# wenet-e2e/wenet

Measured on AMD Instinct MI355X. Metric: audio-seconds/sec (RTF^-1), 12L Conformer fbank80, ctc_prefix_beam_search, higher is better.
Workload: dtype f32 (feed-forward and subsampling-conv2 GEMMs: fp32 operands as three exact bf16 planes, six plane products on the bf16 matrix cores, f32 accumulate -- error <= the v_mfma_f32 kernel's, tests/test_gpu_x6.py; everything else v_mfma_f32)

## Files before the change

### wenet_amd/csrc/ffn_x6f.hip

```cpp
#include <type_traits>

#include "common.h"
#include "gemm_epilogue.h"
#include "kernels.h"
#include "x6.h"

namespace wn {

namespace {

__device__ unsigned long long g_x6f_clk[4][24];

constexpr int REC = X3_REC;
constexpr int XSTAGE = 24 * REC;
constexpr int XD = 256;
constexpr int XKB = XD / 16;

typedef unsigned u32x4 __attribute__((ext_vector_type(4)));
struct Frag6 { bf16x8 p[2][3]; };

__global__ __launch_bounds__(256) void x6_split_perm_kernel(const float* __restrict__ src, int R,
                                                            int K, int ld,
                                                            char* __restrict__ dst) {
  const int tiles = (R + 31) >> 5, nkb = K >> 4;
  const int64_t idx = (int64_t)blockIdx.x * 256 + threadIdx.x;
  const int row_l = (int)(idx & 31), h = (int)((idx >> 5) & 1);
  const int64_t rest = idx >> 6;
  const int kb = (int)(rest % nkb), tile = (int)(rest / nkb);
  if (tile >= tiles) return;
  const int row = tile * 32 + row_l;
  f32x4 a = {0.f, 0.f, 0.f, 0.f}, b = a;
  if (row < R) {
    const float* s = src + (int64_t)row * ld + kb * 16 + h * 4;
    a = *reinterpret_cast<const f32x4*>(s);
    b = *reinterpret_cast<const f32x4*>(s + 8);
  }
  bf16x8 p0, p1, p2;
#pragma unroll
  for (int e = 0; e < 4; ++e) {
    const Split3 sa = split3(a[e]), sb = split3(b[e]);
    p0[e] = sa.h0; p1[e] = sa.h1; p2[e] = sa.h2;
    p0[4 + e] = sb.h0; p1[4 + e] = sb.h1; p2[4 + e] = sb.h2;
  }
  char* o = dst + ((int64_t)kb * tiles + tile) * X3_TILE + h * 512 + row_l * 16;
  *reinterpret_cast<bf16x8*>(o) = p0;
  *reinterpret_cast<bf16x8*>(o + REC) = p1;
  *reinterpret_cast<bf16x8*>(o + 2 * REC) = p2;
}

__device__ __forceinline__ void wait_vm_stages(int stages) {
  switch (stages) {
    case 0: asm volatile("s_waitcnt vmcnt(0)" ::: "memory"); break;
    case 1: asm volatile("s_waitcnt vmcnt(6)" ::: "memory"); break;
    case 2: asm volatile("s_waitcnt vmcnt(12)" ::: "memory"); break;
    case 3: asm volatile("s_waitcnt vmcnt(18)" ::: "memory"); break;
    default: asm volatile("s_waitcnt vmcnt(24)" ::: "memory"); break;
  }
}

template <int ACT, int RING, int VAR>
__global__ __launch_bounds__(256, 1) void ffn_x6f_kernel(FfnX6Args p, int tiles_m, int pairmap) {
  extern __shared__ __attribute__((aligned(16))) char smem_g[];
  typedef __attribute__((address_space(3))) void* lds_ptr;
  constexpr int HALF = (VAR & 512) ? 2 : 1;
  constexpr int STG = XSTAGE * HALF;
  constexpr int SPC = 8 / HALF;
  static_assert(RING >= 3 && RING * STG <= 6 * XSTAGE, "ring of at most 144 KB");
  float* b1s = reinterpret_cast<float*>(smem_g + RING * STG);

  const int bid = blockIdx.x, xcd = bid & 7, rr = bid >> 3;
  int slice, tm;
  if (pairmap && p.S >= 2 && p.S <= 8) {
    const int nsp = p.S >> 1, pair = xcd % nsp, tg = xcd / nsp;
    slice = 2 * pair + (rr & 1);
    tm = (rr >> 1) * (8 / nsp) + tg;
  } else if (p.S <= 8) {
    slice = xcd & (p.S - 1);
    tm = rr * (8 / p.S) + xcd / p.S;
  } else {
    const int sub = p.S >> 3;
    slice = xcd + 8 * (rr % sub);
    tm = rr / sub;
  }
  if (tm >= tiles_m) return;

  unsigned long long clk[20] = {0, 0, 0, 0, 0, 0, 0, 0, 0, 0, 0, 0, 0, 0, 0, 0, 0, 0, 0, 0};
  if constexpr ((VAR & 8192) != 0) {
    clk[9] = __builtin_readcyclecounter();
    clk[12] = __builtin_amdgcn_s_memrealtime();
  }
  const int tid = threadIdx.x, lane = tid & 63;
  const int wave = __builtin_amdgcn_readfirstlane(tid >> 6);
  __builtin_assume(wave >= 0 && wave < 4);
  const int hi = lane >> 5, li = lane & 31;
  const int NC = p.F / p.S / 64;
  const int cg0 = slice * NC;
  const int FT = p.F >> 5;
  const unsigned vlane = (unsigned)lane * 16u;

  const __amdgpu_buffer_rsrc_t r1 = __builtin_amdgcn_make_buffer_rsrc(
      const_cast<char*>(reinterpret_cast<const char*>(p.W13)), 0,
      (int)((int64_t)p.F * XD * 6), 0x00020000);
  const __amdgpu_buffer_rsrc_t r2 = __builtin_amdgcn_make_buffer_rsrc(
      const_cast<char*>(reinterpret_cast<const char*>(p.W2p)), 0,
      (int)((int64_t)p.F * XD * 6), 0x00020000);

  auto issue_sub = [&](int c, int sub, int buf) {
    char* dst = smem_g + buf * STG + (sub % HALF) * XSTAGE + wave * 6 * REC;
    const int cg = cg0 + c;
    if (sub < 4) {
      const int nt = sub >> 1;
#pragma unroll
      for (int j2 = 0; j2 < 2; ++j2) {
        const int ks = (sub & 1) * 8 + wave * 2 + j2;
        const int so = ((ks * FT + 2 * cg + nt) * 3) * REC;
#pragma unroll
        for (int pl = 0; pl < 3; ++pl)
          __builtin_amdgcn_raw_ptr_buffer_load_lds(r1, (lds_ptr)(dst + (j2 * 3 + pl) * REC), 16,
                                                   vlane, so + pl * REC, 0, 0);
      }
    } else {
      const int so = ((cg * 4 + sub - 4) * 24 + wave * 6) * REC;
#pragma unroll
      for (int j = 0; j < 6; ++j)
        __builtin_amdgcn_raw_ptr_buffer_load_lds(r2, (lds_ptr)(dst + j * REC), 16, vlane,
                                                 so + j * REC, 0, 0);
    }
  };
  auto issue = [&](int c, int st, int buf) {
#pragma unroll
    for (int h = 0; h < HALF; ++h) issue_sub(c, st * HALF + h, buf);
  };
  auto issue_one = [&](int c, int sub, int buf, int j) {
    char* dst = smem_g + buf * STG + (sub % HALF) * XSTAGE + wave * 6 * REC + j * REC;
    const int cg = cg0 + c;
    if (sub < 4) {
      const int nt = sub >> 1, j2 = j / 3, pl = j - j2 * 3;
      const int ks = (sub & 1) * 8 + wave * 2 + j2;
      const int so = ((ks * FT + 2 * cg + nt) * 3) * REC;
      __builtin_amdgcn_raw_ptr_buffer_load_lds(r1, (lds_ptr)dst, 16, vlane, so + pl * REC, 0, 0);
    } else {
      const int so = ((cg * 4 + sub - 4) * 24 + wave * 6) * REC;
      __builtin_amdgcn_raw_ptr_buffer_load_lds(r2, (lds_ptr)dst, 16, vlane, so + j * REC, 0, 0);
    }
  };
  auto read_group = [&](int buf, int g) {
    const char* st = smem_g + buf * STG + g * 6 * REC + lane * 16;
    Frag6 f;
#pragma unroll
    for (int t = 0; t < 2; ++t)
#pragma unroll
      for (int pl = 0; pl < 3; ++pl)
        f.p[t][pl] = *reinterpret_cast<const bf16x8*>(st + (t * 3 + pl) * REC);
    return f;
  };

  constexpr bool XT = (VAR & 16384) != 0;
  constexpr bool XI = (VAR & 32768) != 0;
  bf16x8 X[XKB][3];
  const int xrow = min(tm * 128 + wave * 32 + li, p.M - 1);
  f32x4 xa[XKB], xb[XKB];
  f32x4 xr[4][8];
  if constexpr (XI) {
    const int tiles = (p.M + 31) >> 5;
    const int tile = min(tm * 4 + wave, tiles - 1);
    const char* xi = reinterpret_cast<const char*>(p.X3) + (int64_t)tile * X3_TILE + lane * 16;
    const int64_t kstr = (int64_t)tiles * X3_TILE;
#pragma unroll
    for (int ks = 0; ks < XKB; ++ks)
#pragma unroll
      for (int pl = 0; pl < 3; ++pl)
        X[ks][pl] = *reinterpret_cast<const bf16x8*>(xi + ks * kstr + pl * REC);
  } else if constexpr (XT) {
    const int r4 = lane >> 4, c16 = lane & 15;
#pragma unroll
    for (int q = 0; q < 4; ++q)
#pragma unroll
      for (int j = 0; j < 8; ++j) {
        const int row = min(tm * 128 + wave * 32 + 4 * j + r4, p.M - 1);
        xr[q][j] = *reinterpret_cast<const f32x4*>(p.X + (int64_t)row * p.ldx + q * 64 + c16 * 4);
      }
  } else {
    const float* xr0 = p.X + (int64_t)xrow * p.ldx + hi * 8;
#pragma unroll
    for (int ks = 0; ks < XKB; ++ks) {
      xa[ks] = *reinterpret_cast<const f32x4*>(xr0 + ks * 16);
      xb[ks] = *reinterpret_cast<const f32x4*>(xr0 + ks * 16 + 4);
    }
  }
#pragma unroll
  for (int t = 0; t < ((VAR & 16384) ? RING - 1 : RING); ++t) issue(0, t, t);
  float b1v[8];
#pragma unroll
  for (int i = 0; i < 8; ++i) b1v[i] = p.b1[cg0 * 64 + min(tid + 256 * i, NC * 64 - 1)];
  if constexpr ((VAR & 8192) != 0) { __builtin_amdgcn_sched_barrier(0); clk[15] = __builtin_readcyclecounter(); __builtin_amdgcn_sched_barrier(0); }
  if constexpr (XT && !XI) {
    char* patch = smem_g + (RING - 1) * STG + wave * (32 * 272);
    const int r4 = lane >> 4, c16 = lane & 15;
#pragma unroll
    for (int q = 0; q < 4; ++q) {
#pragma unroll
      for (int j = 0; j < 8; ++j)
        *reinterpret_cast<f32x4*>(patch + (4 * j + r4) * 272 + c16 * 16) = xr[q][j];
#pragma unroll
      for (int k4 = 0; k4 < 4; ++k4) {
        xa[4 * q + k4] = *reinterpret_cast<const f32x4*>(patch + li * 272 + k4 * 64 + hi * 32);
        xb[4 * q + k4] = *reinterpret_cast<const f32x4*>(patch + li * 272 + k4 * 64 + hi * 32 + 16);
      }
      asm volatile("s_waitcnt lgkmcnt(0)" ::: "memory");
    }
  }
  if constexpr (!XI) {
#pragma unroll
    for (int ks = 0; ks < XKB; ++ks) {
#pragma unroll
      for (int e = 0; e < 4; ++e) {
        const Split3 sa = split3(xa[ks][e]), sb = split3(xb[ks][e]);
        X[ks][0][e] = sa.h0; X[ks][1][e] = sa.h1; X[ks][2][e] = sa.h2;
        X[ks][0][4 + e] = sb.h0; X[ks][1][4 + e] = sb.h1; X[ks][2][4 + e] = sb.h2;
      }
    }
  }
  if constexpr ((VAR & 8192) != 0) { __builtin_amdgcn_sched_barrier(0); clk[16] = __builtin_readcyclecounter(); __builtin_amdgcn_sched_barrier(0); }
  asm volatile("s_waitcnt vmcnt(0)" ::: "memory");
  if constexpr ((VAR & 8192) != 0) { __builtin_amdgcn_sched_barrier(0); clk[17] = __builtin_readcyclecounter(); __builtin_amdgcn_sched_barrier(0); }
#pragma unroll
  for (int ks = 0; ks < XKB; ++ks)
#pragma unroll
    for (int pl = 0; pl < 3; ++pl) asm volatile("" : "+v"(X[ks][pl]));
#pragma unroll
  for (int i = 0; i < 8; ++i)
    if (tid + 256 * i < NC * 64) b1s[tid + 256 * i] = b1v[i];
  __syncthreads();
  if constexpr ((VAR & 8192) != 0) { __builtin_amdgcn_sched_barrier(0); clk[18] = __builtin_readcyclecounter(); __builtin_amdgcn_sched_barrier(0); }

  f32x16 Y[8];
#pragma unroll
  for (int i = 0; i < 8; ++i)
#pragma unroll
    for (int r = 0; r < 16; ++r) Y[i][r] = 0.f;
  f32x16 HE[2], HO[2];
  u32x4 Hp[4][3];
  if (VAR & 4)
#pragma unroll
    for (int i = 0; i < 12; ++i) {
      Hp[i / 3][i % 3] = u32x4{0x3f803f80u, 0x3f803f80u, 0x3f803f80u, 0x3f803f80u};
      asm volatile("" : "+v"(Hp[i / 3][i % 3]));
    }

  constexpr int PW[6] = {2, 0, 1, 1, 0, 0}, PX[6] = {0, 2, 1, 0, 1, 0};
  constexpr int RT[6] = {0, 1, 0, 1, 0, 1}, RP[6] = {2, 2, 0, 0, 1, 1};

  float pv0 = 0.f, pv1 = 0.f, pt0 = 0.f, pt1 = 0.f;
  unsigned ph0 = 0, ph1 = 0;
  auto pk = [](float a, float b) {
    typedef __bf16 bf16x2 __attribute__((ext_vector_type(2)));
    const bf16x2 h = {(__bf16)a, (__bf16)b};
    return __builtin_bit_cast(unsigned, h);
  };
  auto lo = [](unsigned u) { return __builtin_bit_cast(float, u << 16); };
  auto hi16 = [](unsigned u) { return __builtin_bit_cast(float, u & 0xffff0000u); };
  auto piece_slice = [&](int nt, int i, int k, const f32x4& bq) {
    const int r = 2 * i;
    switch (k) {
      case 0: {
        float b0 = bq[r & 3];
        asm volatile("" : "+v"(b0));
        pv0 = HE[nt][r] + b0;
        break;
      }
      case 1: {
        float b1 = bq[(r + 1) & 3];
        asm volatile("" : "+v"(b1), "+v"(pv0));
        pv0 += HO[nt][r];
        pv1 = HE[nt][r + 1] + b1;
        break;
      }
      case 2:
        asm volatile("" : "+v"(pv0), "+v"(pv1));
        pv1 += HO[nt][r + 1];
        if (ACT == ACT_SILU) pt0 = pv0 * -1.4426950408889634f;
        break;
      case 3:
        if (ACT == ACT_SILU) {
          asm volatile("" : "+v"(pt0), "+v"(pv1));
          pt1 = pv1 * -1.4426950408889634f;
          pt0 = wn_exp2(pt0);
        }
        break;
      case 4:
        if (ACT == ACT_SILU) {
          asm volatile("" : "+v"(pt0), "+v"(pt1));
          pt1 = wn_exp2(pt1);
          pt0 = 1.0f + pt0;
        }
        break;
      case 5:
        if (ACT == ACT_SILU) {
          asm volatile("" : "+v"(pt0), "+v"(pt1));
          pt1 = 1.0f + pt1;
          pt0 = wn_rcp(pt0);
        }
        break;
      case 6:
        asm volatile("" : "+v"(pv0));
        if (ACT == ACT_SILU) {
          asm volatile("" : "+v"(pt0), "+v"(pt1));
          pt1 = wn_rcp(pt1);
          pv0 *= pt0;
        }
        if (ACT == ACT_RELU) pv0 = fmaxf(pv0, 0.0f);
        break;
      case 7:
        asm volatile("" : "+v"(pv0), "+v"(pv1));
        if (ACT == ACT_SILU) {
          asm volatile("" : "+v"(pt1));
          pv1 *= pt1;
        }
        if (ACT == ACT_RELU) pv1 = fmaxf(pv1, 0.0f);
        ph0 = pk(pv0, pv1);
        break;
      case 8:
        asm volatile("" : "+v"(pv0), "+v"(pv1), "+v"(ph0));
        pv0 -= lo(ph0); pv1 -= hi16(ph0);
        break;
      case 9:
        asm volatile("" : "+v"(pv0), "+v"(pv1));
        ph1 = pk(pv0, pv1);
        break;
      case 10:
        asm volatile("" : "+v"(pv0), "+v"(pv1), "+v"(ph1));
        pv0 -= lo(ph1); pv1 -= hi16(ph1);
        break;
      default: {
        asm volatile("" : "+v"(pv0), "+v"(pv1));
        const int kb = 2 * nt + (r >> 3), d = (r & 7) >> 1;
        Hp[kb][0][d] = ph0;
        Hp[kb][1][d] = ph1;
        Hp[kb][2][d] = pk(pv0, pv1);
        break;
      }
    }
  };
  auto read_frag = [&](int b, int g, int t, int pl) {
    return *reinterpret_cast<const bf16x8*>(smem_g + b * STG + (g * 6 + t * 3 + pl) * REC +
                                            lane * 16);
  };
  const f32x16 zero16 = {0.f, 0.f, 0.f, 0.f, 0.f, 0.f, 0.f, 0.f, 0.f, 0.f, 0.f, 0.f, 0.f, 0.f, 0.f,
                         0.f};

  int buf = 0;
  Frag6 fc;
#pragma unroll
  for (int q = 0; q < 6; ++q) fc.p[RT[q]][RP[q]] = read_frag(0, 0, RT[q], RP[q]);
  if constexpr ((VAR & 8192) != 0) clk[10] = __builtin_readcyclecounter();
  auto chunk = [&](auto last_tag, int c) {
    constexpr bool last = decltype(last_tag)::value;
    f32x4 bq = {0.f, 0.f, 0.f, 0.f};
#pragma unroll
    for (int sub = 0; sub < 8; ++sub) {
      if constexpr ((VAR & 8192) != 0 && !last) {
        __builtin_amdgcn_sched_barrier(0);
        clk[sub] = __builtin_readcyclecounter();
        __builtin_amdgcn_sched_barrier(0);
      }
#pragma unroll
      for (int g = 0; g < 4; ++g) {
        Frag6 fn;
        const bool do_piece = sub >= 2 && sub < 6;
        const int pnt = sub >= 4 ? 1 : 0;
        const int pi = ((sub & 1) << 2) + g;
        if (do_piece && (pi & 1) == 0)
          bq = *reinterpret_cast<const f32x4*>(b1s + c * 64 + pnt * 32 + 8 * (pi >> 1) + 4 * hi);
#pragma unroll
        for (int k = 0; k < 12; ++k) {
          const int q = k >> 1, tl = k & 1;
          if ((VAR & 1) || ((VAR & 65536) && q >= 3)) {
            asm volatile("" ::"v"(fc.p[tl][PW[q]]));
          } else if (sub < 4) {
            const int nt = sub >> 1, ks = (sub & 1) * 8 + 2 * g + tl;
            const bool first = (sub & 1) == 0 && g == 0 && q == 0;
            f32x16& H = tl == 0 ? HE[nt] : HO[nt];
            H = __builtin_amdgcn_mfma_f32_32x32x16_bf16(fc.p[tl][PW[q]], X[ks][PX[q]],
                                                       first ? zero16 : H, 0, 0, 0);
          } else {
            const bf16x8 hb = __builtin_bit_cast(bf16x8, Hp[sub - 4][PX[q]]);
            Y[2 * g + tl] = __builtin_amdgcn_mfma_f32_32x32x16_bf16(fc.p[tl][PW[q]], hb,
                                                                    Y[2 * g + tl], 0, 0, 0);
          }
          const int st = sub / HALF;
          const bool sync_sub = sub % HALF == HALF - 1;
          const int gs = (sub % HALF) * 4 + g;
          if (g == 3 && k == 5 && sync_sub) {
            __builtin_amdgcn_sched_barrier(0);
            if (!(VAR & 8)) {
              if (!(VAR & 1024)) {
                asm volatile("s_waitcnt lgkmcnt(0)" ::: "memory");
                const int tail = SPC - 2 - st < 0 ? 0 : (SPC - 2 - st > RING - 2 ? RING - 2 : SPC - 2 - st);
                if (last) wait_vm_stages(tail * HALF); else wait_vm_stages((RING - 2) * HALF);
              }
              if (!(VAR & 2048)) __builtin_amdgcn_s_barrier();
            }
            if (!(VAR & 2) && !(VAR & 16384)) {
              if (st + RING < SPC) issue(c, st + RING, buf);
              else if (!last) issue(c + 1, st + RING - SPC, buf);
            }
            buf = buf + 1 == RING ? 0 : buf + 1;
            __builtin_amdgcn_sched_barrier(0);
          }
          if constexpr ((VAR & 16384) != 0 && !(VAR & 2)) {
            static_assert(!(VAR & 16384) || HALF == 2, "spread DMA: 48-record stages");
            const int ka = do_piece ? 9 : 2, kb = do_piece ? 11 : 8;
            if ((k == ka || k == kb) && gs < 6) {
              const int j12 = gs * 2 + (k == kb ? 1 : 0);
              const int tst = st + RING - 1;
              const int bufp = buf == 0 ? RING - 1 : buf - 1;
              if (tst < SPC) issue_one(c, tst * HALF + j12 / 6, bufp, j12 % 6);
              else if (!last) issue_one(c + 1, (tst - SPC) * HALF + j12 / 6, bufp, j12 % 6);
            }
          }
          if (VAR & 64) {
            fn = fc;
          } else if (g < 3 || !sync_sub) {
            if (VAR & 4096) {
              if (k == 0)
#pragma unroll
                for (int i = 0; i < 6; ++i) fn.p[RT[i]][RP[i]] = read_frag(buf, gs + 1, RT[i], RP[i]);
            } else if (tl == 1) {
              fn.p[RT[q]][RP[q]] = read_frag(buf, gs + 1, RT[q], RP[q]);
            }
          } else if (k >= 6 && (sub < 7 || !last)) {
            fn.p[RT[k - 6]][RP[k - 6]] = read_frag(buf, 0, RT[k - 6], RP[k - 6]);
          }
          if (do_piece) {
            if (VAR & 4) {
              if (k == 11) {
                const int r = 2 * pi, kb = 2 * pnt + (r >> 3), d = (r & 7) >> 1;
                Hp[kb][0][d] = __builtin_bit_cast(unsigned, HE[pnt][r]) & 0x3f803f80u;
                Hp[kb][1][d] = __builtin_bit_cast(unsigned, HO[pnt][r]) & 0x3f803f80u;
                Hp[kb][2][d] = __builtin_bit_cast(unsigned, HE[pnt][r + 1]) & 0x3f803f80u;
              }
            } else {
              piece_slice(pnt, pi, k, bq);
            }
          }
          __builtin_amdgcn_sched_barrier(0);
        }
        fc = fn;
      }
    }
    if constexpr ((VAR & 8192) != 0 && !last) clk[8] = __builtin_readcyclecounter();
  };
  for (int c = 0; c + 1 < NC; ++c) chunk(std::false_type{}, c);
  chunk(std::true_type{}, NC - 1);

  if constexpr ((VAR & 8192) != 0) clk[11] = __builtin_readcyclecounter();
  const int row = tm * 128 + wave * 32 + li;
  if constexpr (XT) {
    __syncthreads();
    char* patch = smem_g + wave * (32 * 1040);
#pragma unroll
    for (int i = 0; i < 8; ++i)
#pragma unroll
      for (int g = 0; g < 4; ++g)
        *reinterpret_cast<f32x4*>(patch + li * 1040 + (i * 32 + 8 * g + 4 * hi) * 4) =
            f32x4{Y[i][4 * g], Y[i][4 * g + 1], Y[i][4 * g + 2], Y[i][4 * g + 3]};
    float* P0 = p.P + ((int64_t)slice * p.M + tm * 128 + wave * 32) * XD + lane * 4;
    const int nrow = min(32, p.M - (tm * 128 + wave * 32));
#pragma unroll
    for (int r = 0; r < 32; ++r) {
      const f32x4 v = *reinterpret_cast<const f32x4*>(patch + r * 1040 + lane * 16);
      if (r < nrow) *reinterpret_cast<f32x4*>(P0 + (int64_t)r * XD) = v;
    }
  } else if (row < p.M) {
    float* P = p.P + ((int64_t)slice * p.M + row) * XD;
#pragma unroll
    for (int i = 0; i < 8; ++i)
#pragma unroll
      for (int g = 0; g < 4; ++g)
      {
        const f32x4 v = f32x4{Y[i][4 * g], Y[i][4 * g + 1], Y[i][4 * g + 2], Y[i][4 * g + 3]};
        float* o = P + i * 32 + 8 * g + 4 * hi;
        if (VAR & 128) asm volatile("global_store_dwordx4 %0, %1, off sc0 sc1" ::"v"(o), "v"(v) : "memory");
        else if (VAR & 256) asm volatile("global_store_dwordx4 %0, %1, off nt" ::"v"(o), "v"(v) : "memory");
        else *reinterpret_cast<f32x4*>(o) = v;
      }
  }
  if constexpr ((VAR & 8192) != 0) {
    asm volatile("s_waitcnt vmcnt(0)" ::: "memory");
    clk[13] = __builtin_amdgcn_s_memrealtime();
    const unsigned long long t_end = __builtin_readcyclecounter();
    if (blockIdx.x == gridDim.x / 2 && lane == 0) {
#pragma unroll
      for (int i = 0; i < 20; ++i) g_x6f_clk[wave][i] = clk[i];
      g_x6f_clk[wave][20] = t_end;
    }
  }
}

template <int ACT, int RING, int VAR = 0>
int launch_x6f(const FfnX6Args& a, hipStream_t s) {
  const int tiles_m = cdiv(a.M, 128);
  const int NC = a.F / a.S / 64;
  const size_t lds = (size_t)RING * XSTAGE * ((VAR & 512) ? 2 : 1) + (size_t)NC * 64 * sizeof(float);
  const int pairmap = a.S >= 2 && a.S <= 8;
  const int grid = pairmap      ? cdiv(tiles_m, 16 / a.S) * 16
                   : a.S <= 8 ? cdiv(tiles_m, 8 / a.S) * 8
                              : tiles_m * a.S;
  auto kern = ffn_x6f_kernel<ACT, RING, VAR>;
  WN_MAX_DYN_LDS(kern, 160 * 1024);
  hipLaunchKernelGGL(kern, dim3(grid), dim3(256), lds, s, a, tiles_m, pairmap);
  WN_HIP(hipGetLastError());
  return 0;
}

}


int ffn_x6f_clocks(unsigned long long* out) {
  WN_HIP(hipMemcpyFromSymbol(out, HIP_SYMBOL(g_x6f_clk), sizeof(g_x6f_clk)));
  return 0;
}

int x6_split_perm(const float* src, int R, int K, int ld, void* dst, hipStream_t s) {
  WN_CHECK(src && dst && R > 0 && K > 0 && K % 16 == 0 && ld % 4 == 0, "x6_split_perm: shape");
  const int64_t n = (int64_t)cdiv(R, 32) * (K / 16) * 64;
  hipLaunchKernelGGL(x6_split_perm_kernel, dim3((unsigned)((n + 255) / 256)), dim3(256), 0, s,
                     src, R, K, ld, reinterpret_cast<char*>(dst));
  WN_HIP(hipGetLastError());
  return 0;
}

int ffn_x6f_split(int M, int F) {
  const int tiles_m = cdiv(M, 128);
  int S = 1;
  while (S < 32 && tiles_m * (S * 2) <= 256 && F % (S * 2 * 64) == 0) S *= 2;
  return S;
}

bool ffn_x6f_supported(int M, int D, int F, int act) {
  if (D != XD || M <= 0 || F <= 0 || F % 64 != 0) return false;
  if (act != ACT_SILU && act != ACT_RELU) return false;
  const int S = ffn_x6f_split(M, F);
  if (F % (S * 64) != 0 || F / S > 2048) return false;
  if ((int64_t)cdiv(M, 32) * X3_TILE * XKB >= ((int64_t)1 << 40)) return false;
  return tune().ffn_x6f != 3 || cdiv(M, 128) * S >= 128;
}

int ffn_x6f(const FfnX6Args& a, hipStream_t s) {
  WN_CHECK((a.X3 || (a.X && a.ldx % 4 == 0)) && a.W13 && a.W2p && a.b1 && a.P && a.M > 0 && a.D == XD && a.S > 0 &&
               a.F % (a.S * 64) == 0 && a.F / a.S <= 2048 && (a.S & (a.S - 1)) == 0 && a.S <= 32,
           "ffn_x6f: bad arguments");
#define WN_X6F(RING, VAR)                                            \
  switch (a.act) {                                                   \
    case ACT_SILU: return launch_x6f<ACT_SILU, RING, VAR>(a, s);     \
    case ACT_RELU: return launch_x6f<ACT_RELU, RING, VAR>(a, s);     \
    default: break;                                                  \
  }
  if (tune().ffn_x6f_var == 25088 && a.act == ACT_SILU) {
    if (a.X3) return launch_x6f<ACT_SILU, 3, 25088 + 32768>(a, s);
    return launch_x6f<ACT_SILU, 3, 25088>(a, s);
  }
#ifdef WN_ABLATION
  if (tune().ffn_x6f_var != 0 && a.act == ACT_SILU) {
    switch (tune().ffn_x6f_var) {
      case 1: return launch_x6f<ACT_SILU, 6, 1>(a, s);
      case 2: return launch_x6f<ACT_SILU, 6, 2>(a, s);
      case 4: return launch_x6f<ACT_SILU, 6, 4>(a, s);
      case 8: return launch_x6f<ACT_SILU, 6, 8>(a, s);
      case 64: return launch_x6f<ACT_SILU, 6, 64>(a, s);
      case 10: return launch_x6f<ACT_SILU, 6, 10>(a, s);
      case 78: return launch_x6f<ACT_SILU, 6, 78>(a, s);
      case 74: return launch_x6f<ACT_SILU, 6, 74>(a, s);
      case 14: return launch_x6f<ACT_SILU, 6, 14>(a, s);
      case 76: return launch_x6f<ACT_SILU, 6, 76>(a, s);
      case 70: return launch_x6f<ACT_SILU, 6, 70>(a, s);
      case 1094: return launch_x6f<ACT_SILU, 6, 1094>(a, s);
      case 4096: return launch_x6f<ACT_SILU, 6, 4096>(a, s);
      case 4110: return launch_x6f<ACT_SILU, 6, 4110>(a, s);
      case 2118: return launch_x6f<ACT_SILU, 6, 2118>(a, s);
      case 128: return launch_x6f<ACT_SILU, 6, 128>(a, s);
      case 8704: return launch_x6f<ACT_SILU, 3, 8704>(a, s);
      case 82432: return launch_x6f<ACT_SILU, 3, 82432>(a, s);
      case 90624: return launch_x6f<ACT_SILU, 3, 90624>(a, s);
      case 512: return launch_x6f<ACT_SILU, 3, 512>(a, s);
      case 8768: return launch_x6f<ACT_SILU, 3, 8768>(a, s);
      case 8708: return launch_x6f<ACT_SILU, 3, 8708>(a, s);
      case 8706: return launch_x6f<ACT_SILU, 3, 8706>(a, s);
      case 8782: return launch_x6f<ACT_SILU, 3, 8782>(a, s);
      default: break;
    }
  }
  if (tune().ffn_x6f_ring == 4) { WN_X6F(4, 0) }
  else if (tune().ffn_x6f_ring == 5) { WN_X6F(5, 0) }
  else if (tune().ffn_x6f_ring >= 6) { WN_X6F(6, 0) }
#endif
  if (a.X3) { WN_X6F(3, 16896 + 32768) }
  WN_X6F(3, 16896)
#undef WN_X6F
  set_error("ffn_x6f: unsupported activation");
  return -1;
}

}
```

### wenet_amd/csrc/tune.h

```cpp
#pragma once
#include <stdint.h>

#include <string>

namespace wn {

#define WN_TUNE_KEYS(X)                                                                         \
                          \
  X(gemm_tile_bf16, 0)                                                                          \
                            \
  X(bf16_store, 1)                                                                              \
                      \
  X(lp_probe, 0)                                                                                \
                       \
  X(attn_split, 0)                                                                              \
                     \
  X(attn_bf16, 1)                                                                               \
                 \
  X(attn_bf16_nw, 0)                                                                            \
                                                                            \
  X(attn_bf16_defer, 80)                                                                        \
                                                              \
  X(attn_bf16_dma, 1)                                                                           \
                        \
  X(qkv_bf16, 1)                                                                                \
            \
  X(fp8_min_tiles, 192)                                                                         \
       \
  X(ffn_fused, 1)                                                                               \
                                                                   \
  X(gemm_x6, 1)                                                                                 \
                                         \
  X(x6_linear, 1)                                                                               \
                      \
  X(x6_af32, 0)                                                                                 \
            \
  X(x6_conv_af32, 0)                                                                            \
     \
  X(enc_gate_pos, 0)                                                                            \
                                                            \
  X(x6_conv_bm, 128)                                                                            \
                    \
  X(x6_probe, 0)                                                                                \
                     \
  X(ffn_x6f, 1)                                                                                 \
            \
  X(ffn_ximg, 1)                                                                                \
                             \
  X(ffn_x6f_ring, 3)                                                                            \
                  \
  X(ffn_x6f_var, 0)                                                                             \
                                                                        \
  X(x6r, 1)                                                                                     \
                  \
  X(x6r_chain, 1)                                                                               \
          \
  X(x6r_dwc, 1)                                                                                 \
        \
  X(x6r_pro, 1)                                                                                 \
            \
  X(x6r512_rows, 0)                                                                             \
                 \
  X(gemm_rowln, 1)                                                                              \
          \
  X(dwconv_tiled, 1)                                                                            \
                               \
  X(attn_x6, 1)                                                                                 \
                   \
  X(attn_xcd, 1)                                                                                \
        \
  X(attn_x6_galign, 2)                                                                          \
                             \
  X(attn_x6_order, 1)                                                                           \
    \
  X(attn_x6_var, 0)                                                                             \
        \
  X(attn_fold, 1)                                                                               \
                  \
  X(rescore_groups, 1)                                                                          \
                                                \
  X(rescore_prefetch, 1)                                                                        \
    \
  X(beam_weak_hash, 0)                                                                          \
                                                                              \
  X(beam_lds_pool, 1)                                                                           \
    \
  X(sync_spin, 1)                                                                               \
                         \
  X(ctc_wave, 1)                                                                                \
        \
  X(dec_skinny, 0)                                                                              \
                                            \
  X(rnnt_lookahead, 4)

struct Tune {
#define X(name, dflt) int name = dflt;
  WN_TUNE_KEYS(X)
#undef X
};

constexpr int32_t TUNE_INHERIT = INT32_MIN;

extern Tune g_tune_default;
extern thread_local const Tune* t_tune;
inline const Tune& tune() { return t_tune ? *t_tune : g_tune_default; }

int* tune_field(Tune& t, const std::string& key);
int tune_check(const std::string& key, int32_t value, const char* who);
void tune_resolve(const Tune& ovr, Tune* eff);
Tune tune_all_inherit();

}
```

Measured before the change: 71040.

## Overlap first-half FFN output store with last chunk's MFMA tail

Adds an EB variant of the x6 FFN kernel that reorders the final chunk's second-GEMM subtiles so the first half of the output Y finishes early. That half is written through a free LDS ring slot and buffer-stored to global memory while the remaining MFMAs run, and the last barrier is skipped. Only the second half goes through the epilogue afterwards, which shortens the serialized store tail. A new tune key ffn_x6f_ends defaults to enabling it; the cost is more register pressure and an LDS slot reuse that depends on the shipped RING=3/HALF=2 stage shape.

```diff
diff --git a/wenet_amd/csrc/ffn_x6f.hip b/wenet_amd/csrc/ffn_x6f.hip
--- a/wenet_amd/csrc/ffn_x6f.hip
+++ b/wenet_amd/csrc/ffn_x6f.hip
@@ -157,6 +157,8 @@
 
   constexpr bool XT = (VAR & 16384) != 0;
   constexpr bool XI = (VAR & 32768) != 0;
+  constexpr bool EB = (VAR & 262144) != 0;
+  static_assert(!EB || (XT && HALF == 2 && RING == 3), "early half store: the shipped stage shape");
   bf16x8 X[XKB][3];
   const int xrow = min(tm * 128 + wave * 32 + li, p.M - 1);
   f32x4 xa[XKB], xb[XKB];
@@ -350,6 +352,44 @@
                          0.f};
 
   int buf = 0;
+  constexpr int EROW = 528;
+  auto ends_perm = [](int n) { return (n & 1) | ((n & 2) << 1) | ((n & 4) >> 1); };
+  char* epatch = smem_g;
+  f32x4 ev[16];
+  const int enrow = __builtin_amdgcn_readfirstlane(max(0, min(32, p.M - (tm * 128 + wave * 32))));
+  const uint64_t ebase = reinterpret_cast<uint64_t>(
+      p.P + ((int64_t)slice * p.M + tm * 128 + wave * 32) * XD);
+  const __amdgpu_buffer_rsrc_t er = __builtin_amdgcn_make_buffer_rsrc(
+      reinterpret_cast<void*>(
+          (uint64_t)(unsigned)__builtin_amdgcn_readfirstlane((int)(unsigned)ebase) |
+          ((uint64_t)(unsigned)__builtin_amdgcn_readfirstlane((int)(unsigned)(ebase >> 32)) << 32)),
+      0, enrow * (XD * 4), 0x00020000);
+  int evoff = 0;
+  auto ends_write = [&](int i0, int w) {
+    const int i = w >> 2, g4 = w & 3;
+    *reinterpret_cast<f32x4*>(epatch + li * EROW + (i * 32 + 8 * g4 + 4 * hi) * 4) =
+        f32x4{Y[i0 + i][4 * g4], Y[i0 + i][4 * g4 + 1], Y[i0 + i][4 * g4 + 2], Y[i0 + i][4 * g4 + 3]};
+  };
+  auto ends_read = [&](int j) {
+    ev[j] = *reinterpret_cast<const f32x4*>(epatch + (2 * j + hi) * EROW + li * 16);
+  };
+  auto ends_store = [&](int i0, int j) {
+    __builtin_amdgcn_raw_buffer_store_b128(__builtin_bit_cast(u32x4, ev[j]), er,
+                                               evoff + j * (2 * XD * 4) + i0 * 128, 0, 0);
+  };
+  auto ends_slot = [&](int s) {
+    if (s == 0) {
+      int d = buf + 1 + (wave >> 1);
+      d = d >= RING ? d - RING : d;
+      epatch = smem_g + d * STG + (wave & 1) * (32 * EROW);
+      evoff = hi * (XD * 4) + li * 16;
+      asm volatile("" : "+v"(evoff));
+    }
+    if (s < 8) { ends_write(0, 2 * s); ends_write(0, 2 * s + 1); }
+    if (s >= 8 && s < 40 && (s & 1) == 0) ends_read((s - 8) >> 1);
+    if (s >= 11 && s < 43 && (s & 1) == 1) ends_store(0, (s - 11) >> 1);
+  };
+
   Frag6 fc;
 #pragma unroll
   for (int q = 0; q < 6; ++q) fc.p[RT[q]][RP[q]] = read_frag(0, 0, RT[q], RP[q]);
@@ -368,6 +408,7 @@
       for (int g = 0; g < 4; ++g) {
         Frag6 fn;
         const bool do_piece = sub >= 2 && sub < 6;
+        const bool reord = EB && last && sub >= 6;
         const int pnt = sub >= 4 ? 1 : 0;
         const int pi = ((sub & 1) << 2) + g;
         if (do_piece && (pi & 1) == 0)
@@ -384,14 +425,15 @@
             H = __builtin_amdgcn_mfma_f32_32x32x16_bf16(fc.p[tl][PW[q]], X[ks][PX[q]],
                                                        first ? zero16 : H, 0, 0, 0);
           } else {
-            const bf16x8 hb = __builtin_bit_cast(bf16x8, Hp[sub - 4][PX[q]]);
-            Y[2 * g + tl] = __builtin_amdgcn_mfma_f32_32x32x16_bf16(fc.p[tl][PW[q]], hb,
-                                                                    Y[2 * g + tl], 0, 0, 0);
+            const int pg = reord ? ends_perm((sub & 1) * 4 + g) : (sub & 1) * 4 + g;
+            const int hk = reord ? 2 + (pg >> 2) : sub - 4, yt = reord ? 2 * (pg & 3) + tl : 2 * g + tl;
+            const bf16x8 hb = __builtin_bit_cast(bf16x8, Hp[hk][PX[q]]);
+            Y[yt] = __builtin_amdgcn_mfma_f32_32x32x16_bf16(fc.p[tl][PW[q]], hb, Y[yt], 0, 0, 0);
           }
           const int st = sub / HALF;
           const bool sync_sub = sub % HALF == HALF - 1;
           const int gs = (sub % HALF) * 4 + g;
-          if (g == 3 && k == 5 && sync_sub) {
+          if (g == 3 && k == 5 && sync_sub && !(reord && sub == 7)) {
             __builtin_amdgcn_sched_barrier(0);
             if (!(VAR & 8)) {
               if (!(VAR & 1024)) {
@@ -427,7 +469,7 @@
 #pragma unroll
                 for (int i = 0; i < 6; ++i) fn.p[RT[i]][RP[i]] = read_frag(buf, gs + 1, RT[i], RP[i]);
             } else if (tl == 1) {
-              fn.p[RT[q]][RP[q]] = read_frag(buf, gs + 1, RT[q], RP[q]);
+              fn.p[RT[q]][RP[q]] = read_frag(buf, reord ? ends_perm(gs + 1) : gs + 1, RT[q], RP[q]);
             }
           } else if (k >= 6 && (sub < 7 || !last)) {
             fn.p[RT[k - 6]][RP[k - 6]] = read_frag(buf, 0, RT[k - 6], RP[k - 6]);
@@ -444,6 +486,7 @@
               piece_slice(pnt, pi, k, bq);
             }
           }
+          if (reord && sub == 7) ends_slot(g * 12 + k);
           __builtin_amdgcn_sched_barrier(0);
         }
         fc = fn;
@@ -456,7 +499,14 @@
 
   if constexpr ((VAR & 8192) != 0) clk[11] = __builtin_readcyclecounter();
   const int row = tm * 128 + wave * 32 + li;
-  if constexpr (XT) {
+  if constexpr (EB) {
+#pragma unroll
+    for (int w = 0; w < 16; ++w) ends_write(4, w);
+#pragma unroll
+    for (int j = 0; j < 16; ++j) ends_read(j);
+#pragma unroll
+    for (int j = 0; j < 16; ++j) ends_store(4, j);
+  } else if constexpr (XT) {
     __syncthreads();
     char* patch = smem_g + wave * (32 * 1040);
 #pragma unroll
@@ -557,7 +607,12 @@
     case ACT_RELU: return launch_x6f<ACT_RELU, RING, VAR>(a, s);     \
     default: break;                                                  \
   }
+  const bool eb = (tune().ffn_x6f_ends & 2) != 0;
   if (tune().ffn_x6f_var == 25088 && a.act == ACT_SILU) {
+    if (eb) {
+      if (a.X3) return launch_x6f<ACT_SILU, 3, 25088 + 32768 + 262144>(a, s);
+      return launch_x6f<ACT_SILU, 3, 25088 + 262144>(a, s);
+    }
     if (a.X3) return launch_x6f<ACT_SILU, 3, 25088 + 32768>(a, s);
     return launch_x6f<ACT_SILU, 3, 25088>(a, s);
   }
@@ -595,6 +650,10 @@
   else if (tune().ffn_x6f_ring == 5) { WN_X6F(5, 0) }
   else if (tune().ffn_x6f_ring >= 6) { WN_X6F(6, 0) }
 #endif
+  if (eb) {
+    if (a.X3) { WN_X6F(3, 16896 + 32768 + 262144) }
+    WN_X6F(3, 16896 + 262144)
+  }
   if (a.X3) { WN_X6F(3, 16896 + 32768) }
   WN_X6F(3, 16896)
 #undef WN_X6F
diff --git a/wenet_amd/csrc/tune.h b/wenet_amd/csrc/tune.h
--- a/wenet_amd/csrc/tune.h
+++ b/wenet_amd/csrc/tune.h
@@ -50,6 +50,8 @@
   X(ffn_x6f_ring, 3)                                                                            \
                   \
   X(ffn_x6f_var, 0)                                                                             \
+        \
+  X(ffn_x6f_ends, 2)                                                                            \
                                                                         \
   X(x6r, 1)                                                                                     \
                   \
```

Result: no change. 70950 (median of 2 runs) (-0.1%).
